# JianCao92/speaker-diarization

Measured on AMD Instinct MI355X. Metric: diarized audio throughput (CD gw/BIC + CL hi/BIC), higher is better.
Workload: dtype f64

## Files before the change

### include/spkd.h

```cpp
#ifndef SPKD_H
#define SPKD_H

#include <stddef.h>
#include <stdint.h>

#ifdef __cplusplus
extern "C" {
#endif

#define SPKD_ABI_VERSION 2
#define SPKD_DIM 39
#define SPKD_REC 820

typedef enum {
    SPKD_OK = 0,
    SPKD_EINVAL = 1,
    SPKD_EHIP = 2,
    SPKD_ENONFINITE = 3,
    SPKD_EOVERFLOW = 4,
    SPKD_ENOMEM = 5
} spkd_status;

typedef enum { SPKD_BIC = 0, SPKD_GLR = 1, SPKD_KL2 = 2, SPKD_KL2_PINV = 3 } spkd_kind;

// ... 165 lines not shown
enum { SPKD_AHC_AUTO = 0, SPKD_AHC_MONO = 1, SPKD_AHC_WIDE = 2 };

typedef struct {
    int32_t variant;
    int32_t kind;
    int32_t max_spk;
    int32_t path;
    double lambdac;
    double threshold;
} spkd_ahc_params;

spkd_status spkd_ahc(spkd_ctx *ctx, const double *d_stats, const int64_t *h_seg_off,
                     int64_t n_problems, const spkd_ahc_params *params,
                     int32_t *h_n_merges, int32_t *h_merge_a, int32_t *h_merge_b,
                     double *h_merge_d, double *h_stat_max, double *h_stat_min);

spkd_status spkd_ahc_matrix(spkd_ctx *ctx, const double *d_stats, int64_t n, const spkd_ahc_params *params,
                            const double *d_matrix, double stat_max_in, double stat_min_in,
                            int32_t *h_n_merges, int32_t *h_merge_a, int32_t *h_merge_b,
                            double *h_merge_d, double *h_stat_max, double *h_stat_min);

spkd_status spkd_ahc_fused(spkd_ctx *ctx, const float *d_frames, int64_t n_frames,
                           const double *d_records, int64_t n_records, int64_t *d_line_index,
                           const int64_t *h_seg_off, int64_t n_problems,
                           const int64_t *h_redo_line, const int64_t *h_redo_begin,
                           const int64_t *h_redo_end, int64_t n_redo,
                           const spkd_ahc_params *params,
                           const int32_t **h_n_merges, const int32_t **h_merge_a,
                           const int32_t **h_merge_b, const double **h_merge_d,
                           const int32_t **h_labels);
// ... 158 lines not shown
```

### speaker-diarization_amd/csrc/spkd_cluster.hpp

```cpp
#pragma once
#include "spkd_device.hpp"
#include "spkd_quad.hpp"
#include "spkd_tri.hpp"
#include "../../include/spkd.h"

namespace spkd {

constexpr double MAXINT_F = 9223372036854775808.0;
constexpr double PEN_UNIT = 39.0 + 0.5 * 39.0 * 40.0;
constexpr int AUX = 3 * DA;
constexpr int ERR_DEGENERATE_MERGE = 2;

__device__ __forceinline__ unsigned long long dkey(double v) {
    unsigned long long b = (unsigned long long)__double_as_longlong(v);
    return (b >> 63) ? ~b : (b | 0x8000000000000000ull);
}
__device__ __forceinline__ double dkey_inv(unsigned long long k) {
    unsigned long long b = (k >> 63) ? (k & 0x7fffffffffffffffull) : ~k;
    return __longlong_as_double((long long)b);
}
template <bool MAXOP>
__device__ __forceinline__ unsigned wave_red_u32(unsigned x) {
    auto op = [](unsigned a, unsigned b) { return MAXOP ? (a > b ? a : b) : (a < b ? a : b); };
    x = op(x, (unsigned)__builtin_amdgcn_update_dpp((int)x, (int)x, 0xB1, 0xf, 0xf, false));
// ... 504 lines not shown
            }
        }
    }
    if (variant == 1 && (kind == SPKD_KL2 ? lane_id() == 0 : L.t == 0)) {
        if (wmax == wmax) atomicMax(stat_max + p, dkey(wmax));
        if (wmin == wmin) atomicMin(stat_min + p, dkey(wmin));
    }
}

constexpr int AHC_WAVES = 8;
constexpr int AHC_TPB = AHC_WAVES * WAVE;

#ifdef SPKD_PROFILE
__device__ unsigned long long g_step_prof[8];
__device__ unsigned long long g_ahc_prof[8];
#endif
constexpr int NO_COL = 0x7fffffff;
constexpr int AHC_MAX_N = 65536;


struct RowMin { double mv; int mc, nc; };

template <class Alive>
__device__ __forceinline__ RowMin scan_row(const double* __restrict__ row, long long N, Alive alive,
                                           long long sub_col, double sub_val, int lane) {
    double mv = __builtin_huge_val();
    int mc = NO_COL, nc = NO_COL;
    for (long long c0 = 0; c0 < N; c0 += 4 * WAVE) {
        double v[4];
        int a[4];
// ... 103 lines not shown
        }
    }
}

template <bool TWO>
__global__ __launch_bounds__(AHC_TPB) void k_ahc(
        double* __restrict__ ex, double* __restrict__ pk, const int64_t* __restrict__ seg_off,
        int variant, int kind, int max_spk, double lambdac, double threshold,
        double* __restrict__ ld, double* __restrict__ aux,
        double* __restrict__ mat, const int64_t* __restrict__ mat_off,
        int32_t* __restrict__ alive, double* __restrict__ tmp,
        double* __restrict__ rmin_all, int32_t* __restrict__ rcache_all,
        int32_t* __restrict__ out_n, int32_t* __restrict__ out_a, int32_t* __restrict__ out_b,
        double* __restrict__ out_d, unsigned long long* stat_max, unsigned long long* stat_min,
        double* __restrict__ final_max, double* __restrict__ final_min, int* err,
        double* pinv_ws) {
    extern __shared__ int32_t ids[];
    __shared__ double ldsA[QREC];
    __shared__ unsigned long long red3[AHC_WAVES][3];
    __shared__ unsigned long long s_masks[AHC_MAX_N / WAVE];
    __shared__ int s_cnt[2];
    __shared__ int s_nids;
    __shared__ int s_next;
    __shared__ double s_tmax[AHC_WAVES];
    const int tid = threadIdx.x, lane = lane_id(), wave = tid >> 6;
    const QuadLane L = quad_lane();
    const int p = blockIdx.x;
    const int64_t off = seg_off[p];
    const long long N = seg_off[p + 1] - off;
    double* Dm = mat + mat_off[p];
    int32_t* al = alive + off;
    double* ldp = ld + off;
    double* tp = tmp + off;
    double* rmin = rmin_all + off;
    int32_t* rarg = rcache_all + 3 * off;
    int32_t* rnan = rarg + N;
    int32_t* dirty = rnan + N;
    for (long long c = tid; c < N; c += AHC_TPB) { al[c] = 1; dirty[c] = 1; }
    __syncthreads();
    long long m = N;
    int n_merges = 0;
    const long long INF_IDX = 0x7fffffffffffffffLL;
// ... 170 lines not shown
                if (kmax != 0ull) atomicMax(stat_max + p, kmax);
                if (kmin != ~0ull) atomicMin(stat_min + p, kmin);
            }
        }
        __syncthreads();
        AHC_TICK(4);
    }
#ifdef SPKD_PROFILE
    if (tid == 0) for (int i = 0; i < 5; ++i) atomicAdd(&g_ahc_prof[2 + i], ahc_acc[i]);
#endif
    const double mx = final_matrix_max(Dm, N, [&](long long c) { return al[c] != 0; }, s_tmax, tid);
    if (tid == 0) {
        out_n[p] = n_merges;
        final_max[p] = mx;
        final_min[p] = fmin;
    }
}

constexpr int STEP_WAVES = 4;
constexpr int STEP_WIDE_FROM = 1024;
constexpr int STEP_PARTNERS = 4 * STEP_WAVES - 1;
constexpr int ALIVE_ROUND = 0x7fffffff;
constexpr int STEP_MAX_N = 16384;
constexpr int STEP_IDX_SHIFT = 14;

struct StepState {
    int32_t done, n_merges;
    long long psa;
    double fmin;
    double diag;
// ... 599 lines not shown
```

### speaker-diarization_amd/csrc/spkd_hip.hip

```cpp
#include <hip/hip_runtime.h>

#include <algorithm>
#include <cmath>
#include <cstddef>
#include <cstdio>
#include <cstdlib>
#include <cstring>
#include <string>
#include <atomic>
#include <thread>
#include <vector>

#include "../../include/spkd.h"
#include "spkd_cd.hpp"
#include "spkd_cluster.hpp"
#include "spkd_device.hpp"
#include "spkd_handoff.hpp"
#include "spkd_merge.hpp"
#include "spkd_stats.hpp"
#include "spkd_post_stats.hpp"
#include "spkd_mfcc.hpp"
#include "spkd_mfcc_batch.hpp"
#include "spkd_resample.hpp"
#include "spkd_vad.hpp"
// ... 14 lines not shown
       PIN_GT_TAB, PIN_GT_OUT, PIN_GT_IDX, PIN_UBM_TAB, PIN_UBM_OUT, PIN_CLR_IN, PIN_CLR_OUT, PIN_MD_SEQS, PIN_MD_TOKENS,
       PIN_FB_TAB, PIN_ID_IN, PIN_ID_OUT, PIN_ACC_TAB, PIN_POST_TAB, N_PIN };
}

struct spkd_ctx {
    int device = 0;
    hipStream_t stream = nullptr;
    bool own_stream = false;
    bool gw_lds_ok = false;
    int rs_lds_cap = 0;
    int gw_waves = 0;
    unsigned long long init_keys[2] = {0ull, ~0ull};
    int step_waves = 0;
    int step_partners = 0;
    int64_t last_gw_items = 0;
    std::string err;
    int* d_err = nullptr;
    unsigned long long* d_counter = nullptr;
    hipEvent_t ev0 = nullptr, ev1 = nullptr;
    float last_ms = 0.f;
    hipEvent_t ka[SPKD_N_TIMERS] = {}, kb[SPKD_N_TIMERS] = {};
    bool kused[SPKD_N_TIMERS] = {};
    float kms[SPKD_N_TIMERS] = {};
    void* slot[N_SLOTS] = {};
    size_t slot_bytes[N_SLOTS] = {};
    void* pinv_ws = nullptr;
    double* pinv_cur = nullptr;
    void* pin[N_PIN] = {};
    size_t pin_bytes[N_PIN] = {};
    std::vector<int64_t> redo_line, redo_begin, redo_end;
// ... 93 lines not shown
template <class Parts>
spkd_status upload_parts(spkd_ctx* c, int slot, std::vector<char>& image, Parts parts) {
    image.resize(parts(Layout()));
    parts(Layout(nullptr, image.data()));
    char* d = nullptr;
    TRY(upload(c, slot, image.data(), image.size(), &d));
    parts(Layout(d));
    return SPKD_OK;
}

struct Call {
    spkd_ctx* const c;
    spkd_status opened;
    int herr = 0;
    bool drained = false;
    explicit Call(spkd_ctx* ctx) : c(ctx) { opened = open(); }
    ~Call() { if (!drained) (void)hipStreamSynchronize(c->stream); }
    spkd_status open() {
        HIPCHK(c, hipSetDevice(c->device));
        for (int i = 0; i < SPKD_N_TIMERS; ++i) c->kused[i] = false;
        HIPCHK(c, hipMemsetAsync(c->d_err, 0, sizeof(int), c->stream));
        HIPCHK(c, hipEventRecord(c->ev0, c->stream));
        return SPKD_OK;
    }

    spkd_status finish() {
        HIPCHK(c, hipEventRecord(c->ev1, c->stream));
        HIPCHK(c, hipMemcpyAsync(&herr, c->d_err, sizeof(int), hipMemcpyDeviceToHost, c->stream));
        HIPCHK(c, hipStreamSynchronize(c->stream));
        drained = true;
        HIPCHK(c, hipEventElapsedTime(&c->last_ms, c->ev0, c->ev1));
        c->kms[0] = c->last_ms;
        for (int i = 1; i < SPKD_N_TIMERS; ++i)
            if (c->kused[i]) HIPCHK(c, hipEventElapsedTime(&c->kms[i], c->ka[i], c->kb[i]));
        if (herr & ERR_SWEEP) return fail(c, SPKD_EHIP, "internal error: growing-window sweep order");
        if (herr & 4) return fail(c, SPKD_EOVERFLOW, "device scratch capacity exceeded");
        if (herr & ERR_DEGENERATE_MERGE) return fail(c, SPKD_EINVAL, "degenerate merge: a diagonal cell was the minimum");
        if (herr & ERR_NONFINITE) return fail(c, SPKD_ENONFINITE, "array must not contain infs or NaNs");
        return SPKD_OK;
    }
};

struct Image { char* base = nullptr; size_t bytes = 0; };
template <class Tab, class Parts>
// ... 106 lines not shown
    c->gw_lds_ok = hipDeviceGetAttribute(&lds_max, hipDeviceAttributeMaxSharedMemoryPerBlock, device) == hipSuccess &&
                   Gw<4>::LDS_BYTES <= lds_max &&
                   hipFuncSetAttribute((const void*)k_gw<8>, hipFuncAttributeMaxDynamicSharedMemorySize, Gw<8>::LDS_BYTES) == hipSuccess &&
                   hipFuncSetAttribute((const void*)k_gw<4>, hipFuncAttributeMaxDynamicSharedMemorySize, Gw<4>::LDS_BYTES) == hipSuccess &&
                   hipFuncSetAttribute((const void*)k_gw<2>, hipFuncAttributeMaxDynamicSharedMemorySize, Gw<2>::LDS_BYTES) == hipSuccess &&
                   hipFuncSetAttribute((const void*)k_gw<1>, hipFuncAttributeMaxDynamicSharedMemorySize, Gw<1>::LDS_BYTES) == hipSuccess;
    c->rs_lds_cap = 64 * 1024;
    if (lds_max > c->rs_lds_cap) {
        const int want = lds_max < RS_LDS_MAX ? lds_max : RS_LDS_MAX;
        if (hipFuncSetAttribute((const void*)k_resample, hipFuncAttributeMaxDynamicSharedMemorySize, want) == hipSuccess)
            c->rs_lds_cap = want;
    }
    if (const char* e = getenv("SPKD_GW_WAVES")) c->gw_waves = atoi(e);
    if (const char* e = getenv("SPKD_STEP_WAVES")) { const int v = atoi(e); c->step_waves = (v == 4 || v == 8) ? v : 0; }
    if (const char* e = getenv("SPKD_STEP_PARTNERS")) { const int v = atoi(e); c->step_partners = (v == 3 || v == 7 || v == 15) ? v : 0; }
    *out = c;
    return SPKD_OK;
}

spkd_status spkd_create(int device, void* stream, spkd_ctx** out) {
    return create_ctx(device, stream, stream != nullptr, out);
}

spkd_status spkd_create_on_stream(int device, void* stream, spkd_ctx** out) {
    return create_ctx(device, stream, true, out);
}

void spkd_destroy(spkd_ctx* c) {
    if (!c) return;
    (void)hipSetDevice(c->device);
    if (c->stream) (void)hipStreamSynchronize(c->stream);
    for (int i = 0; i < N_SLOTS; ++i)
        if (c->slot[i]) (void)hipFree(c->slot[i]);
    if (c->d_err) (void)hipFree(c->d_err);
    if (c->pinv_ws) (void)hipFree(c->pinv_ws);
    for (int i = 0; i < N_PIN; ++i)
        if (c->pin[i]) (void)hipHostFree(c->pin[i]);
    if (c->d_counter) (void)hipFree(c->d_counter);
    if (c->ev0) (void)hipEventDestroy(c->ev0);
    if (c->ev1) (void)hipEventDestroy(c->ev1);
    for (int i = 0; i < SPKD_N_TIMERS; ++i) {
        if (c->ka[i]) (void)hipEventDestroy(c->ka[i]);
        if (c->kb[i]) (void)hipEventDestroy(c->kb[i]);
    }
    if (c->own_stream && c->stream) (void)hipStreamDestroy(c->stream);
    delete c;
// ... 142 lines not shown
namespace {
struct AhcPrep {
    double* ex;
    double* pk;
    double* ld;
    double* aux;
    double* mat;
    int64_t* seg_off;
    int64_t* mat_off;
    unsigned long long* smax;
    unsigned long long* smin;
    int64_t n_total = 0;
    int64_t grid_rows = 0;
    std::vector<char> offs;
    std::vector<char> prob_of;
};

unsigned long long host_dkey(double v) {
    unsigned long long b;
    std::memcpy(&b, &v, sizeof b);
    return (b >> 63) ? ~b : (b | 0x8000000000000000ull);
}

struct MatrixPlan {
    const double* d_init = nullptr;
    double init_max = NAN, init_min = NAN;
    int64_t row_begin = -1, row_end = -1;
    int64_t* d_map = nullptr;
    int64_t n_src = 0;
    const float* d_frames = nullptr;
    int64_t n_frames = 0;
    const int64_t *redo_line = nullptr, *redo_begin = nullptr, *redo_end = nullptr;
    int64_t n_redo = 0;
};

void to_quadrec(spkd_ctx* c, const double* d_stats, int64_t n, double* ex) {
    hipLaunchKernelGGL(k_to_quadrec, dim3((unsigned)n), dim3(256), 0, c->stream, d_stats, n, ex);
}

void cluster_prep(spkd_ctx* c, const double* ex, int64_t n, int kind, double* ld, double* aux) {
    const int64_t per_block = kind == SPKD_KL2 ? PT_WAVES : 4 * PT_WAVES;
    const unsigned blocks = (unsigned)((n + per_block - 1) / per_block);
    hipLaunchKernelGGL(k_cluster_prep, dim3(blocks), dim3(PT_WAVES * WAVE), 0, c->stream, ex, n, kind, ld, aux, c->d_err,
                       c->pinv_cur);
}

spkd_status ahc_prepare(spkd_ctx* c, const double* d_stats, const int64_t* h_seg_off, int64_t n_prob,
                        int variant, int kind, double lambdac, AhcPrep& B, const MatrixPlan& plan = MatrixPlan()) {
    const int64_t n_total = B.n_total = h_seg_off[n_prob];
    const size_t np = (size_t)n_prob;
    std::vector<int64_t> mat_off(np + 1);
    int64_t cells = 0;
    for (int64_t p = 0; p < n_prob; ++p) {
        const int64_t n = h_seg_off[p + 1] - h_seg_off[p];
        if (n < 0) return fail(c, SPKD_EINVAL, "seg_off must be non-decreasing");
        mat_off[(size_t)p] = cells;
        cells += n * n;
    }
    mat_off[np] = cells;
    std::vector<int32_t> prob((size_t)n_total, 0);
    for (int64_t p = 0; p < n_prob; ++p)
        for (int64_t r = h_seg_off[p]; r < h_seg_off[p + 1]; ++r) prob[(size_t)r] = (int32_t)p;
    int32_t *d_prob = nullptr, *d_sched = nullptr;
    {
        const int X = 8;
        std::vector<std::vector<int32_t>> lists(X);
        if (plan.row_begin >= 0) {
            for (int64_t r = plan.row_begin; r < plan.row_end; ++r) lists[(size_t)((r - plan.row_begin) % X)].push_back((int32_t)r);
        } else if (n_prob >= X) {
            std::vector<int64_t> order((size_t)n_prob);
            for (int64_t p = 0; p < n_prob; ++p) order[(size_t)p] = p;
            std::stable_sort(order.begin(), order.end(), [&](int64_t a, int64_t b) {
                return h_seg_off[a + 1] - h_seg_off[a] > h_seg_off[b + 1] - h_seg_off[b];
            });
            double load[X] = {0, 0, 0, 0, 0, 0, 0, 0};
            for (int64_t p : order) {
                int x = 0;
                for (int i = 1; i < X; ++i) if (load[i] < load[x]) x = i;
                const double n = (double)(h_seg_off[p + 1] - h_seg_off[p]);
                load[x] += n * n;
                for (int64_t r = h_seg_off[p]; r < h_seg_off[p + 1]; ++r) lists[x].push_back((int32_t)r);
            }
        } else {
            for (int64_t r = 0; r < n_total; ++r) lists[(size_t)(r % X)].push_back((int32_t)r);
        }
        size_t longest = 0;
        for (auto& l : lists) longest = std::max(longest, l.size());
        B.grid_rows = (int64_t)longest * X;
        std::vector<int32_t> sched((size_t)B.grid_rows, -1);
        for (int x = 0; x < X; ++x)
            for (size_t i = 0; i < lists[x].size(); ++i) sched[i * X + x] = lists[x][i];
        TRY(upload_parts(c, S_AHC_OFF, B.offs, [&](Layout L) {
            return L.part(B.seg_off, np + 1, h_seg_off).part(B.mat_off, np + 1, mat_off.data()).bytes();
        }));
        TRY(upload_parts(c, S_AHC_PROB, B.prob_of, [&](Layout L) {
            return L.part(d_prob, prob.size(), prob.data()).part(d_sched, sched.size(), sched.data()).bytes();
        }));
    }
    const size_t nt = (size_t)n_total;
    TRY(carve(c, scratch, S_AHC_LD, [&](Layout L) { return L.part(B.ld, nt).bytes(); }));
    TRY(carve(c, scratch, S_AHC_AUX, [&](Layout L) { return L.part(B.aux, nt * AUX).bytes(); }));
    TRY(carve(c, scratch, S_AHC_MAT, [&](Layout L) { return L.part(B.mat, (size_t)cells).bytes(); }));
    TRY(carve(c, scratch, S_AHC_MISC, [&](Layout L) { return L.part(B.smax, np).part(B.smin, np).bytes(); }));
    HIPCHK(c, hipMemsetAsync(B.smax, 0x00, (size_t)n_prob * sizeof(unsigned long long), c->stream));
    HIPCHK(c, hipMemsetAsync(B.smin, 0xff, (size_t)n_prob * sizeof(unsigned long long), c->stream));
    if (plan.d_init && n_prob == 1) {
        c->init_keys[0] = plan.init_max == plan.init_max ? host_dkey(plan.init_max) : 0ull;
        c->init_keys[1] = plan.init_min == plan.init_min ? host_dkey(plan.init_min) : ~0ull;
        HIPCHK(c, hipMemcpyAsync(B.smax, &c->init_keys[0], sizeof(unsigned long long), hipMemcpyHostToDevice, c->stream));
        HIPCHK(c, hipMemcpyAsync(B.smin, &c->init_keys[1], sizeof(unsigned long long), hipMemcpyHostToDevice, c->stream));
    }
    TRY(carve(c, scratch, S_AHC_STATS, [&](Layout L) { return L.part(B.ex, nt * QREC).bytes(); }));
    TRY(carve(c, scratch, S_AHC_PACKED, [&](Layout L) { return L.part(B.pk, nt * REC).bytes(); }));
// ... 9 lines not shown
                TRY(set_stats_launch(c, plan.d_frames, plan.n_frames, plan.redo_begin, plan.redo_end, c->redo_sets.data(),
                                     plan.n_redo, plan.n_redo, (double*)d_redo, c->redo_chunks, c->redo_setoff));
                hipLaunchKernelGGL(k_patch_map, dim3((unsigned)((plan.n_redo + 255) / 256)), dim3(256), 0, c->stream,
                                   (const int64_t*)d_rl, plan.n_redo, plan.d_map);
            }
            hipLaunchKernelGGL(k_records_from_map, dim3((unsigned)n_total), dim3(256), 0, c->stream, d_stats, plan.n_src,
                               (const int64_t*)plan.d_map, (const double*)d_redo, plan.n_redo, n_total, B.ex, B.pk, c->d_err);
        } else {
            to_quadrec(c, d_stats, n_total, B.ex);
            HIPCHK(c, hipMemcpyAsync(B.pk, d_stats, (size_t)n_total * REC * sizeof(double), hipMemcpyDeviceToDevice, c->stream));
        }
        {
            Timer t(c, SPKD_T_CLUSTER_PREP);
            cluster_prep(c, B.ex, n_total, kind, B.ld, B.aux);
        }
        auto kmat = kind == SPKD_GLR ? k_matrix<true> : k_matrix<false>;
        if (plan.d_init) {
            HIPCHK(c, hipMemcpyAsync(B.mat, plan.d_init, (size_t)cells * sizeof(double), hipMemcpyDeviceToDevice, c->stream));
        } else if (B.grid_rows > 0) {
            Timer t(c, SPKD_T_MATRIX);
            hipLaunchKernelGGL(kmat, dim3((unsigned)B.grid_rows), dim3(MX_WAVES * WAVE), 0, c->stream,
                               (const double*)B.ex, (const double*)B.pk, (const int64_t*)B.seg_off, (const int32_t*)d_prob,
                               (const int32_t*)d_sched, variant, kind, lambdac,
                               (const double*)B.ld, (const double*)B.aux, B.mat, (const int64_t*)B.mat_off,
                               B.smax, B.smin, c->d_err);
        }
    }
    HIPCHK(c, hipGetLastError());
    return SPKD_OK;
}

double key_to_double(unsigned long long k, bool is_max) {
    if (is_max ? (k == 0ull) : (k == ~0ull)) return std::nan("");
    unsigned long long b = (k >> 63) ? (k & 0x7fffffffffffffffull) : ~k;
    double v;
    std::memcpy(&v, &b, sizeof v);
    return v;
}
}

// ... 192 lines not shown
        return fail(c, SPKD_EINVAL, "null argument");
    if ((P->variant != 1 && P->variant != 2) || bad_kind(P->kind))
        return fail(c, SPKD_EINVAL, "bad variant / kind");
    for (int64_t p = 0; p < n_prob; ++p)
        if (h_seg_off[p + 1] - h_seg_off[p] < 1) return fail(c, SPKD_EINVAL, "empty clustering problem");
    int64_t n_max = 0;
    for (int64_t p = 0; p < n_prob; ++p) n_max = std::max<int64_t>(n_max, h_seg_off[p + 1] - h_seg_off[p]);
    if (n_max > AHC_MAX_N) return fail(c, SPKD_EINVAL, "clustering problem larger than 65536 records");
    int path = P->path;
    if (path != SPKD_AHC_MONO && path != SPKD_AHC_WIDE) path = n_prob <= 64 ? SPKD_AHC_WIDE : SPKD_AHC_MONO;
    const size_t lds = (size_t)(n_max + 4) * sizeof(int32_t);
    if (path == SPKD_AHC_MONO && lds > 150 * 1024) path = SPKD_AHC_WIDE;
    if (path == SPKD_AHC_WIDE && n_max > STEP_MAX_N)
        return fail(c, SPKD_EINVAL, "clustering problem larger than 16384 records (wide merge loop)");
    AhcPrep B;
    std::vector<unsigned long long> kmax((size_t)n_prob), kmin((size_t)n_prob);
    std::vector<double> fmax((size_t)n_prob), fmin((size_t)n_prob);
    Call call(c);
    TRY(call.opened);
    spkd_ahc_params Pk;
    TRY(kernel_params(c, P, Pk));
    TRY(ahc_prepare(c, d_stats, h_seg_off, n_prob, P->variant, P->kind, P->lambdac, B, plan));
    const int64_t n_total = B.n_total;
    const size_t nt = (size_t)n_total, np = (size_t)n_prob;
    double *d_merge_d, *d_tmp, *d_rmin, *d_fmax, *d_fmin;
    int32_t *d_a, *d_b, *d_alive, *d_rcache, *d_n;
    TRY(carve(c, scratch, S_AHC_OUT, [&](Layout L) {
        return L.part(d_merge_d, nt).part(d_tmp, nt).part(d_rmin, nt).part(d_fmax, np).part(d_fmin, np)
            .part(d_a, nt).part(d_b, nt).part(d_alive, nt).part(d_rcache, 3 * nt).part(d_n, np).bytes();
    }));
    if (path == SPKD_AHC_MONO) {
        auto kahc = P->kind == SPKD_GLR ? k_ahc<true> : k_ahc<false>;
        if (lds > 48 * 1024)
            (void)hipFuncSetAttribute((const void*)kahc, hipFuncAttributeMaxDynamicSharedMemorySize, (int)lds);
        Timer t(c, SPKD_T_AHC);
        hipLaunchKernelGGL(kahc, dim3((unsigned)n_prob), dim3(AHC_TPB), lds, c->stream,
                           B.ex, B.pk, (const int64_t*)B.seg_off, P->variant, P->kind, P->max_spk, P->lambdac,
                           P->threshold, B.ld, B.aux, B.mat, (const int64_t*)B.mat_off, d_alive, d_tmp,
                           d_rmin, d_rcache, d_n, d_a, d_b, d_merge_d, B.smax, B.smin, d_fmax, d_fmin, c->d_err,
                           c->pinv_cur);
    } else {
        StepArrays Q;
        void *pe = nullptr, *pp = nullptr;
        TRY(carve(c, scratch, S_STEP_MISC, [&](Layout L) {
            return L.part(Q.sel2, 2 * nt).part(Q.cnt, nt).part(Q.sw, nt).part(Q.state2, 2 * np).part(Q.death, nt).bytes();
        }));
        TRY(scratch(c, S_STEP_EXM, nt * QREC * sizeof(double), &pe));
        TRY(scratch(c, S_STEP_PKM, nt * REC * sizeof(double), &pp));
        Q.ex = B.ex; Q.pk = B.pk; Q.exm = (double*)pe; Q.pkm = (double*)pp;
        Q.n_total = n_total;
        Q.n_prob = (int32_t)n_prob;
        const int step_waves = c->step_waves ? c->step_waves : (n_max > STEP_WIDE_FROM ? 8 : 4);
        const bool glr_k = P->kind == SPKD_GLR;
        using StepKernel = decltype(&k_ahc_step<false, 4, 3>);
        StepKernel kvar[3];
// ... 66 lines not shown
                    h_stat_max, h_stat_min);
}

spkd_status spkd_ahc_matrix(spkd_ctx* c, const double* d_stats, int64_t n, const spkd_ahc_params* P,
                            const double* d_matrix, double stat_max_in, double stat_min_in,
                            int32_t* h_n_merges, int32_t* h_merge_a, int32_t* h_merge_b, double* h_merge_d,
                            double* h_stat_max, double* h_stat_min) {
    if (!c || n < 1) return SPKD_EINVAL;
    if (!d_matrix) return fail(c, SPKD_EINVAL, "ahc_matrix: null matrix");
    const int64_t seg_off[2] = {0, n};
    MatrixPlan plan;
    plan.d_init = d_matrix;
    plan.init_max = stat_max_in;
    plan.init_min = stat_min_in;
    return ahc_impl(c, d_stats, seg_off, 1, P, plan, h_n_merges, h_merge_a, h_merge_b, h_merge_d, h_stat_max, h_stat_min);
}

int64_t spkd_gw_event_capacity(int64_t turn_len, double rate) {
    if (turn_len < 0 || !(rate >= 10.0)) return -1;
    return (int64_t)((double)turn_len / (0.2 * rate)) + 8;
}

int64_t spkd_gw_event_capacity_p(int64_t turn_len, const spkd_cd_params* P) {
    if (turn_len < 0 || !P || !(P->rate >= 10.0) || !(P->winstep >= 1.0)) return -1;
    const double step = std::min(0.2 * P->rate, std::min(0.5 * P->rate, P->winstep));
    return (int64_t)((double)turn_len / step) + 8;
}

int64_t spkd_sw_window_count(int64_t turn_len, double winsize, double winstep) {
    if (!(winstep >= 1.0) || !(winsize >= 1.0)) return -1;
// ... 2157 lines not shown
        for (auto& th : pool) th.join();
    }
    return bad.load() ? SPKD_EINVAL : SPKD_OK;
}

}

#ifdef SPKD_PROFILE
extern "C" int spkd_debug_ahc_prof(unsigned long long* out4) {
    unsigned long long z[8] = {0, 0, 0, 0, 0, 0, 0, 0};
    if (hipMemcpyFromSymbol(out4, HIP_SYMBOL(spkd::g_ahc_prof), sizeof z) != hipSuccess) return 1;
    if (hipMemcpyToSymbol(HIP_SYMBOL(spkd::g_ahc_prof), z, sizeof z) != hipSuccess) return 1;
    return 0;
}

extern "C" int spkd_debug_step_prof(unsigned long long* out8) {
    unsigned long long z[8] = {0, 0, 0, 0, 0, 0, 0, 0};
    if (hipMemcpyFromSymbol(out8, HIP_SYMBOL(spkd::g_step_prof), sizeof z) != hipSuccess) return 1;
    if (hipMemcpyToSymbol(HIP_SYMBOL(spkd::g_step_prof), z, sizeof z) != hipSuccess) return 1;
    return 0;
}

extern "C" int spkd_debug_pass_prof(unsigned long long* out4) {
    unsigned long long z[4] = {0, 0, 0, 0};
    if (hipMemcpyFromSymbol(out4, HIP_SYMBOL(spkd::g_pass_prof), sizeof z) != hipSuccess) return 1;
    if (hipMemcpyToSymbol(HIP_SYMBOL(spkd::g_pass_prof), z, sizeof z) != hipSuccess) return 1;
    return 0;
}

extern "C" int spkd_debug_gw_prof(unsigned long long* out12) {
// ... 7 lines not shown
```

### speaker-diarization_amd/hipabi.py

```python
import ctypes as C
import os

import numpy as np

HERE = os.path.dirname(os.path.abspath(__file__))
LIB_PATH = os.environ.get('SPKD_HIP_LIBRARY') or os.path.join(HERE, 'csrc', 'libspkd_hip.so')

SPKD_OK, SPKD_EINVAL, SPKD_EHIP, SPKD_ENONFINITE, SPKD_EOVERFLOW, SPKD_ENOMEM = range(6)
KINDS = {'BIC': 0, 'GLR': 1, 'KL2': 2, 'KL2P': 3}
WANT_GLR, WANT_KL2, WANT_KL2_PINV = 1, 2, 4
MERGE_NO_AHEAD = 1
TIMERS = {n: i for i, n in enumerate(['call', 'chunk_stats', 'reduce_sets', 'pair_terms',
                                        'cluster_prep', 'matrix', 'ahc', 'gw', 'sw', 'merge',
                                        'vad_shift', 'vad_viterbi', 'vad_backtrack', 'gauss_models', 'gauss_loglik',
                                        'post_stats', 'resample',
                                        'gmm_train', 'gmm_seq_loglik', 'ubm_stats', 'clr_link',
                                        'mindur_viterbi', 'mindur_backtrack', 'fb_posterior',
                                        'ident_scores', 'ident_assign', 'bw_accumulate',
                                        'mfcc_static', 'mfcc_post'])}
VAD_TILE = 32
MINDUR_TILE = 32
FB_TILE = 32
POST_CHUNK = 1024
GAUSS_TILE = 64
# ... 8 lines not shown
MFCC_POST_TILE = 128
MFCC_POST_HALO = 4
MFCC_POST_LDS = 61440
MFCC_CMS_MAX = 272
RESAMPLE_TILE = 2048
RESAMPLE_MAX_CH = 8
RESAMPLE_MAX_HALF = 256
RESAMPLE_MAX_TERM = 1 << 20
RESAMPLE_MAX_TAPS = 1 << 22
RESAMPLE_MAX_SPAN = 33281
REC = 820
DIM = 39

EXPORTS = ['spkd_abi_version', 'spkd_create', 'spkd_create_on_stream', 'spkd_destroy', 'spkd_last_error', 'spkd_sync',
           'spkd_malloc', 'spkd_free', 'spkd_memcpy_h2d', 'spkd_memcpy_d2h', 'spkd_memcpy_d2d',
           'spkd_last_kernel_ms', 'spkd_last_gw_items', 'spkd_set_stats', 'spkd_pair_terms',
           'spkd_distance_matrix', 'spkd_gw_event_capacity', 'spkd_gw_event_capacity_p', 'spkd_gw', 'spkd_gw_ex', 'spkd_gw_fused', 'spkd_gw_batch', 'spkd_ahc_fused', 'spkd_gather_stats', 'spkd_sum_stats', 'spkd_mfcc', 'spkd_mfcc_batch', 'spkd_resample_batch',
           'spkd_sw_window_count', 'spkd_sw', 'spkd_sw_runs', 'spkd_sw_batch', 'spkd_merge_batch', 'spkd_ahc', 'spkd_ahc_matrix', 'spkd_distance_rows', 'spkd_cluster_in', 'spkd_cluster_in_batch', 'spkd_py2_roundtrip',
           'spkd_labels_from_merges', 'spkd_labels_from_merges_batch', 'spkd_count_flags', 'spkd_gw_lines',
           'spkd_gmm_loglik', 'spkd_vad_viterbi', 'spkd_vad_shift_batch', 'spkd_vad_viterbi_batch',
           'spkd_gauss_models', 'spkd_gauss_loglik', 'spkd_gmm_train', 'spkd_gmm_loglik_seq',
           'spkd_ubm_stats', 'spkd_clr_link', 'spkd_mindur_viterbi_batch', 'spkd_fb_posterior_batch',
           'spkd_clr_identify', 'spkd_bw_accumulate', 'spkd_post_stats']


class CdParams(C.Structure):
    _fields_ = [('kind', C.c_int32), ('trace', C.c_int32), ('lambdac', C.c_double),
                ('threshold', C.c_double), ('winsize', C.c_double), ('winstep', C.c_double),
                ('deltaws', C.c_double), ('rate', C.c_double)]


# ... 100 lines not shown
    lib.spkd_abi_version.restype = C.c_int
    lib.spkd_create.argtypes = [C.c_int, vp, P(vp)]
    lib.spkd_create_on_stream.argtypes = [C.c_int, vp, P(vp)]
    lib.spkd_destroy.argtypes = [vp]
    lib.spkd_destroy.restype = None
    lib.spkd_last_error.argtypes = [vp]
    lib.spkd_last_error.restype = C.c_char_p
    lib.spkd_sync.argtypes = [vp]
    lib.spkd_malloc.argtypes = [vp, C.c_size_t, P(vp)]
    lib.spkd_free.argtypes = [vp, vp]
    lib.spkd_memcpy_h2d.argtypes = [vp, vp, vp, C.c_size_t]
    lib.spkd_memcpy_d2h.argtypes = [vp, vp, vp, C.c_size_t]
    lib.spkd_memcpy_d2d.argtypes = [vp, vp, vp, C.c_size_t]
    lib.spkd_last_kernel_ms.argtypes = [vp, C.c_int, P(C.c_float)]
    lib.spkd_last_gw_items.argtypes = [vp, P(C.c_int64)]
    lib.spkd_set_stats.argtypes = [vp, vp, i64, vp, vp, vp, i64, i64, vp]
    lib.spkd_pair_terms.argtypes = [vp, vp, vp, vp, i64, C.c_int, vp]
    lib.spkd_distance_matrix.argtypes = [vp, C.c_int, dbl, vp, i64, vp]
    lib.spkd_gw_event_capacity.argtypes = [i64, dbl]
    lib.spkd_gw_event_capacity.restype = i64
    lib.spkd_gw_event_capacity_p.argtypes = [i64, P(CdParams)]
    lib.spkd_gw_event_capacity_p.restype = i64
    lib.spkd_gw.argtypes = [vp, vp, i64, vp, vp, i64, P(CdParams), vp, vp, vp, vp, vp, vp, vp, vp,
                            vp, i64, P(i64)]
    lib.spkd_gw_ex.argtypes = [vp, vp, i64, vp, vp, i64, P(CdParams), vp, C.c_int, vp, vp, vp, vp, vp, vp,
                               vp, vp, i64, P(i64)]
    lib.spkd_gw_fused.argtypes = [vp, vp, i64, vp, vp, i64, P(CdParams), vp, C.c_int, vp, vp, vp, vp, vp, vp,
                                  vp, vp, vp, i64, P(i64)]
    lib.spkd_gw_batch.argtypes = [vp, vp, i64, vp, vp, i64, P(CdParams), vp, vp, vp, vp, vp, vp, C.c_int, P(GwLinesView)]
    lib.spkd_ahc_fused.argtypes = [vp, vp, i64, vp, i64, vp, vp, i64, vp, vp, vp, i64, P(AhcParams),
# ... 197 lines not shown
    def check(self, st, allow=()):
        if st != SPKD_OK and st not in allow:
            raise SpkdError(st, self.lib.spkd_last_error(self.h).decode())
        return st

    def last_ms(self, which='call'):
        ms = C.c_float()
        self.check(self.lib.spkd_last_kernel_ms(self.h, TIMERS[which], C.byref(ms)))
        return ms.value

    def last_gw_items(self):
        n = C.c_int64()
        self.check(self.lib.spkd_last_gw_items(self.h, C.byref(n)))
        return int(n.value)

    def dev_alloc(self, nbytes):
        p = C.c_void_p()
        self.check(self.lib.spkd_malloc(self.h, nbytes, C.byref(p)))
        return p.value

    def dev_free(self, ptr):
        if ptr:
            self.check(self.lib.spkd_free(self.h, C.c_void_p(ptr)))

    def dev_scratch(self, name, nbytes):
        cache = self.__dict__.setdefault('_dev_scratch', {})
        ptr, cap = cache.get(name, (None, 0))
        if ptr is None or cap < nbytes:
            if ptr is not None:
                self.dev_free(ptr)
# ... 534 lines not shown
```

### speaker-diarization_amd/pipeline.py

```python
import time

import numpy as np

from . import gallery as _gallery
from . import hipabi
from . import resegmentation as _resegmentation
from .recipe import py2_float_str
from .resegmentation import (FB_MAX_SCALED_PENALTY, RESEG, RESEG_CONF, RESEG_GMM, RESEG_MAX_SPEAKERS, RESEG_MD,
                             RESEG_SOFT, RESEG_SOFT_SCALE, resegment_batch)

DIA2_CD = dict(kind='BIC', lambdac=1.0, threshold=0.0, winsize_s=1.0, winstep_s=3.0, deltaws_s=0.1)
DIA2_CL = dict(variant=1, kind='BIC', lambdac=1.3, threshold=0.0, max_spk=0)
SW_CD = dict(method='sw', kind='GLR', lambdac=1.3, threshold=0.0, winsize_s=5.0, winstep_s=0.5, deltaws_s=0.05)
MERGE_CD = dict(method='m', kind='GLR', lambdac=1.3, threshold=0.0, winsize_s=5.0, winstep_s=0.5, deltaws_s=0.05)
LINK_CL = dict(variant=1, kind='BIC', lambdac=1.3, threshold=0.0, max_spk=0)
LINK_CLR = dict(model='clr', components=8, iterations=5, var_floor=0.01, relevance=16.0,
                threshold=-0.5, max_spk=0, ubm_max_frames=2_000_000)


class BatchFile(object):

    def __init__(self, frame_off, n_frames, vad):
        self.frame_off = int(frame_off)
        self.n_frames = int(n_frames)
# ... 151 lines not shown


def _time_stats(ctx, timings, n, begin, end):
    if len(begin):
        timings.setdefault('chunk_stats', []).append(ctx.last_ms('chunk_stats'))
        timings.setdefault('reduce_sets', []).append(ctx.last_ms('reduce_sets'))
    timings['stats_frames'] = int((end - begin).sum())
    timings['stats_sets'] = n
    timings['stats_recomputed'] = len(begin)


def _clustering_done(ctx, timings, seg_off, r):
    if timings is not None:
        for k in ('cluster_prep', 'matrix', 'ahc'):
            timings.setdefault(k, []).append(ctx.last_ms(k))
    if r['status'] == hipabi.SPKD_ENONFINITE:
        raise ValueError('array must not contain infs or NaNs')
    if timings is not None:
        npb = np.diff(seg_off)
        nm = r['n_merges'].astype(np.int64)
        timings['matrix_pairs'] = int((npb * (npb - 1) // 2).sum())
        timings['ahc_pairs'] = int((nm * (npb - 2) - nm * (nm - 1) // 2).sum())


def _cluster_in_done(ctx, timings, seg_off, r):
    if timings is not None:
        for k in ('cluster_prep', 'ahc'):
            timings.setdefault(k, []).append(ctx.last_ms(k))
    if r['status'] == hipabi.SPKD_ENONFINITE:
        raise ValueError('array must not contain infs or NaNs')
# ... 583 lines not shown
```

Baseline: 1482.

## Overlap head-problem merge loops with remaining distance-matrix build on a side stream

Problems are sorted by size and a host cost model picks a head of the largest ones. Their distance-matrix rows are built first, and their AHC merge loops then start on a second stream. That work overlaps with the matrix build and merge loops for the remaining problems on the main stream. The aim is to stop the long serial merge loop of the biggest problem from sitting idle behind the whole matrix kernel. The cost is extra streams, events and schedule tables, a hard-coded per-N² cost model that may pick a head size of zero, and contention for compute units while the two streams run together.

```diff
diff --git a/include/spkd.h b/include/spkd.h
--- a/include/spkd.h
+++ b/include/spkd.h
@@ -203,6 +203,9 @@
                      int64_t n_problems, const spkd_ahc_params *params,
                      int32_t *h_n_merges, int32_t *h_merge_a, int32_t *h_merge_b,
                      double *h_merge_d, double *h_stat_max, double *h_stat_min);
+
+int64_t spkd_ahc_head_rule(const int64_t *h_seg_off, int64_t n_problems);
+spkd_status spkd_last_ahc_head(spkd_ctx *ctx, int64_t *k);
 
 spkd_status spkd_ahc_matrix(spkd_ctx *ctx, const double *d_stats, int64_t n, const spkd_ahc_params *params,
                             const double *d_matrix, double stat_max_in, double stat_min_in,
diff --git a/speaker-diarization_amd/csrc/spkd_cluster.hpp b/speaker-diarization_amd/csrc/spkd_cluster.hpp
--- a/speaker-diarization_amd/csrc/spkd_cluster.hpp
+++ b/speaker-diarization_amd/csrc/spkd_cluster.hpp
@@ -542,6 +542,8 @@
 #ifdef SPKD_PROFILE
 __device__ unsigned long long g_step_prof[8];
 __device__ unsigned long long g_ahc_prof[8];
+constexpr int AHC_SPAN_PROBS = 4096;
+__device__ unsigned long long g_ahc_span[2 * AHC_SPAN_PROBS];
 #endif
 constexpr int NO_COL = 0x7fffffff;
 constexpr int AHC_MAX_N = 65536;
@@ -675,7 +677,7 @@
         int32_t* __restrict__ out_n, int32_t* __restrict__ out_a, int32_t* __restrict__ out_b,
         double* __restrict__ out_d, unsigned long long* stat_max, unsigned long long* stat_min,
         double* __restrict__ final_max, double* __restrict__ final_min, int* err,
-        double* pinv_ws) {
+        double* pinv_ws, const int32_t* __restrict__ prob_of_block) {
     extern __shared__ int32_t ids[];
     __shared__ double ldsA[QREC];
     __shared__ unsigned long long red3[AHC_WAVES][3];
@@ -686,7 +688,10 @@
     __shared__ double s_tmax[AHC_WAVES];
     const int tid = threadIdx.x, lane = lane_id(), wave = tid >> 6;
     const QuadLane L = quad_lane();
-    const int p = blockIdx.x;
+    const int p = prob_of_block ? prob_of_block[blockIdx.x] : (int)blockIdx.x;
+#ifdef SPKD_PROFILE
+    if (tid == 0 && p < AHC_SPAN_PROBS) g_ahc_span[2 * p] = wall_clock64();
+#endif
     const int64_t off = seg_off[p];
     const long long N = seg_off[p + 1] - off;
     double* Dm = mat + mat_off[p];
@@ -887,6 +892,9 @@
         out_n[p] = n_merges;
         final_max[p] = mx;
         final_min[p] = fmin;
+#ifdef SPKD_PROFILE
+        if (p < AHC_SPAN_PROBS) g_ahc_span[2 * p + 1] = wall_clock64();
+#endif
     }
 }
 
diff --git a/speaker-diarization_amd/csrc/spkd_hip.hip b/speaker-diarization_amd/csrc/spkd_hip.hip
--- a/speaker-diarization_amd/csrc/spkd_hip.hip
+++ b/speaker-diarization_amd/csrc/spkd_hip.hip
@@ -6,6 +6,7 @@
 #include <cstdio>
 #include <cstdlib>
 #include <cstring>
+#include <functional>
 #include <string>
 #include <atomic>
 #include <thread>
@@ -52,6 +53,10 @@
     int step_waves = 0;
     int step_partners = 0;
     int64_t last_gw_items = 0;
+    int ahc_head = -1;
+    int64_t last_ahc_head = 0;
+    hipStream_t side = nullptr;
+    hipEvent_t ev_fork = nullptr, ev_join = nullptr;
     std::string err;
     int* d_err = nullptr;
     unsigned long long* d_counter = nullptr;
@@ -175,8 +180,13 @@
     spkd_status opened;
     int herr = 0;
     bool drained = false;
+    bool forked = false, joined = false;
     explicit Call(spkd_ctx* ctx) : c(ctx) { opened = open(); }
-    ~Call() { if (!drained) (void)hipStreamSynchronize(c->stream); }
+    ~Call() {
+        if (drained) return;
+        (void)hipStreamSynchronize(c->stream);
+        if (forked) (void)hipStreamSynchronize(c->side);
+    }
     spkd_status open() {
         HIPCHK(c, hipSetDevice(c->device));
         for (int i = 0; i < SPKD_N_TIMERS; ++i) c->kused[i] = false;
@@ -185,10 +195,29 @@
         return SPKD_OK;
     }
 
+    spkd_status fork() {
+        if (!c->side) HIPCHK(c, hipStreamCreateWithFlags(&c->side, hipStreamNonBlocking));
+        if (!c->ev_fork) HIPCHK(c, hipEventCreateWithFlags(&c->ev_fork, hipEventDisableTiming));
+        if (!c->ev_join) HIPCHK(c, hipEventCreateWithFlags(&c->ev_join, hipEventDisableTiming));
+        HIPCHK(c, hipEventRecord(c->ev_fork, c->stream));
+        forked = true;
+        HIPCHK(c, hipStreamWaitEvent(c->side, c->ev_fork, 0));
+        return SPKD_OK;
+    }
+    spkd_status join() {
+        if (!forked || joined) return SPKD_OK;
+        HIPCHK(c, hipEventRecord(c->ev_join, c->side));
+        HIPCHK(c, hipStreamWaitEvent(c->stream, c->ev_join, 0));
+        joined = true;
+        return SPKD_OK;
+    }
+
     spkd_status finish() {
+        TRY(join());
         HIPCHK(c, hipEventRecord(c->ev1, c->stream));
         HIPCHK(c, hipMemcpyAsync(&herr, c->d_err, sizeof(int), hipMemcpyDeviceToHost, c->stream));
         HIPCHK(c, hipStreamSynchronize(c->stream));
+        if (forked) HIPCHK(c, hipStreamSynchronize(c->side));
         drained = true;
         HIPCHK(c, hipEventElapsedTime(&c->last_ms, c->ev0, c->ev1));
         c->kms[0] = c->last_ms;
@@ -325,6 +354,7 @@
     if (const char* e = getenv("SPKD_GW_WAVES")) c->gw_waves = atoi(e);
     if (const char* e = getenv("SPKD_STEP_WAVES")) { const int v = atoi(e); c->step_waves = (v == 4 || v == 8) ? v : 0; }
     if (const char* e = getenv("SPKD_STEP_PARTNERS")) { const int v = atoi(e); c->step_partners = (v == 3 || v == 7 || v == 15) ? v : 0; }
+    if (const char* e = getenv("SPKD_AHC_HEAD")) { const int v = atoi(e); c->ahc_head = v >= 0 ? v : -1; }
     *out = c;
     return SPKD_OK;
 }
@@ -341,6 +371,12 @@
     if (!c) return;
     (void)hipSetDevice(c->device);
     if (c->stream) (void)hipStreamSynchronize(c->stream);
+    if (c->side) {
+        (void)hipStreamSynchronize(c->side);
+        (void)hipStreamDestroy(c->side);
+    }
+    if (c->ev_fork) (void)hipEventDestroy(c->ev_fork);
+    if (c->ev_join) (void)hipEventDestroy(c->ev_join);
     for (int i = 0; i < N_SLOTS; ++i)
         if (c->slot[i]) (void)hipFree(c->slot[i]);
     if (c->d_err) (void)hipFree(c->d_err);
@@ -513,7 +549,49 @@
     int64_t grid_rows = 0;
     std::vector<char> offs;
     std::vector<char> prob_of;
+    int64_t head_k = 0;
+    int64_t grid_head = 0;
+    int64_t n_max_head = 0, n_max_rest = 0;
+    int32_t *d_prob = nullptr, *d_sched = nullptr, *d_sched_head = nullptr, *d_block_head = nullptr, *d_block_rest = nullptr;
+    int variant = 1, kind = 0;
+    double lambdac = 0.0;
 };
+
+constexpr int N_XCD = 8;
+void deal_to_xcds(const int64_t* h_seg_off, const std::vector<int64_t>& order, std::vector<int32_t>& sched,
+                  std::vector<int32_t>* by_xcd = nullptr) {
+    const int X = N_XCD;
+    std::vector<std::vector<int32_t>> lists(X), probs(X);
+    if ((int64_t)order.size() >= X) {
+        double load[X] = {0, 0, 0, 0, 0, 0, 0, 0};
+        for (int64_t p : order) {
+            int x = 0;
+            for (int i = 1; i < X; ++i) if (load[i] < load[x]) x = i;
+            const double n = (double)(h_seg_off[p + 1] - h_seg_off[p]);
+            load[x] += n * n;
+            probs[x].push_back((int32_t)p);
+            for (int64_t r = h_seg_off[p]; r < h_seg_off[p + 1]; ++r) lists[x].push_back((int32_t)r);
+        }
+    } else {
+        std::vector<int64_t> asc(order);
+        std::sort(asc.begin(), asc.end());
+        int64_t i = 0;
+        for (size_t k = 0; k < order.size(); ++k) {
+            probs[k].push_back((int32_t)order[k]);
+            for (int64_t r = h_seg_off[asc[k]]; r < h_seg_off[asc[k] + 1]; ++r) lists[(size_t)(i++ % X)].push_back((int32_t)r);
+        }
+    }
+    size_t longest = 0;
+    for (auto& l : lists) longest = std::max(longest, l.size());
+    sched.assign(longest * X, -1);
+    for (int x = 0; x < X; ++x)
+        for (size_t i = 0; i < lists[x].size(); ++i) sched[i * X + x] = lists[x][i];
+    if (by_xcd) {
+        by_xcd->clear();
+        for (size_t i = 0; by_xcd->size() < order.size(); ++i)
+            for (int x = 0; x < X; ++x) if (i < probs[x].size()) by_xcd->push_back(probs[x][i]);
+    }
+}
 
 unsigned long long host_dkey(double v) {
     unsigned long long b;
@@ -544,6 +622,40 @@
                        c->pinv_cur);
 }
 
+void matrix_launch(spkd_ctx* c, const AhcPrep& B, const int32_t* d_sched, int64_t grid) {
+    if (grid <= 0) return;
+    auto kmat = B.kind == SPKD_GLR ? k_matrix<true> : k_matrix<false>;
+    hipLaunchKernelGGL(kmat, dim3((unsigned)grid), dim3(MX_WAVES * WAVE), 0, c->stream,
+                       (const double*)B.ex, (const double*)B.pk, (const int64_t*)B.seg_off, (const int32_t*)B.d_prob,
+                       d_sched, B.variant, B.kind, B.lambdac,
+                       (const double*)B.ld, (const double*)B.aux, B.mat, (const int64_t*)B.mat_off,
+                       B.smax, B.smin, c->d_err);
+}
+
+constexpr int AHC_HEAD_ROUND = 32;
+constexpr double AHC_MS_PER_N2 = 2.095e-4;
+constexpr double MATRIX_MS_PER_N2 = 6.00e-7;
+constexpr int AHC_HEAD_MAX = 32;
+constexpr int AHC_RULE_CUS = 256;
+int64_t ahc_head_rule(const std::vector<int64_t>& n, int cus) {
+    const int64_t n_prob = (int64_t)n.size();
+    if (n_prob < 16) return 0;
+    auto t = [](int64_t N) { return AHC_MS_PER_N2 * (double)N * (double)N; };
+    double sum_all = 0.0;
+    for (int64_t N : n) sum_all += (double)N * (double)N;
+    const double stage0 = MATRIX_MS_PER_N2 * sum_all + t(n[0]);
+    double best = stage0, sum_head = 0.0;
+    int64_t best_k = 0;
+    for (int64_t k = 1; k <= std::min<int64_t>(AHC_HEAD_MAX, n_prob) && k < cus; ++k) {
+        sum_head += (double)n[(size_t)k - 1] * (double)n[(size_t)k - 1];
+        const double m_head = MATRIX_MS_PER_N2 * sum_head, m_rest = MATRIX_MS_PER_N2 * (sum_all - sum_head);
+        const double rest = k < n_prob ? m_rest * cus / (double)(cus - k) + t(n[(size_t)k]) : 0.0;
+        const double stage = m_head + std::max(t(n[0]), rest);
+        if (k % AHC_HEAD_ROUND == 0 && stage < best) { best = stage; best_k = k; }
+    }
+    return stage0 - best < 0.01 * stage0 ? 0 : best_k;
+}
+
 spkd_status ahc_prepare(spkd_ctx* c, const double* d_stats, const int64_t* h_seg_off, int64_t n_prob,
                         int variant, int kind, double lambdac, AhcPrep& B, const MatrixPlan& plan = MatrixPlan()) {
     const int64_t n_total = B.n_total = h_seg_off[n_prob];
@@ -560,42 +672,41 @@
     std::vector<int32_t> prob((size_t)n_total, 0);
     for (int64_t p = 0; p < n_prob; ++p)
         for (int64_t r = h_seg_off[p]; r < h_seg_off[p + 1]; ++r) prob[(size_t)r] = (int32_t)p;
-    int32_t *d_prob = nullptr, *d_sched = nullptr;
     {
-        const int X = 8;
-        std::vector<std::vector<int32_t>> lists(X);
+        std::vector<int32_t> sched, sched_head, block_head, block_rest;
         if (plan.row_begin >= 0) {
-            for (int64_t r = plan.row_begin; r < plan.row_end; ++r) lists[(size_t)((r - plan.row_begin) % X)].push_back((int32_t)r);
-        } else if (n_prob >= X) {
+            const int64_t rows = plan.row_end - plan.row_begin;
+            sched.assign((size_t)((rows + N_XCD - 1) / N_XCD * N_XCD), -1);
+            for (int64_t i = 0; i < rows; ++i) sched[(size_t)i] = (int32_t)(plan.row_begin + i);
+        } else {
             std::vector<int64_t> order((size_t)n_prob);
             for (int64_t p = 0; p < n_prob; ++p) order[(size_t)p] = p;
             std::stable_sort(order.begin(), order.end(), [&](int64_t a, int64_t b) {
                 return h_seg_off[a + 1] - h_seg_off[a] > h_seg_off[b + 1] - h_seg_off[b];
             });
-            double load[X] = {0, 0, 0, 0, 0, 0, 0, 0};
-            for (int64_t p : order) {
-                int x = 0;
-                for (int i = 1; i < X; ++i) if (load[i] < load[x]) x = i;
-                const double n = (double)(h_seg_off[p + 1] - h_seg_off[p]);
-                load[x] += n * n;
-                for (int64_t r = h_seg_off[p]; r < h_seg_off[p + 1]; ++r) lists[x].push_back((int32_t)r);
+            const std::vector<int64_t> head(order.begin(), order.begin() + B.head_k), rest(order.begin() + B.head_k, order.end());
+            deal_to_xcds(h_seg_off, rest, sched);
+            if (B.head_k > 0) {
+                deal_to_xcds(h_seg_off, head, sched_head, &block_head);
+                std::vector<char> in_head((size_t)n_prob, 0);
+                for (int64_t p : head) in_head[(size_t)p] = 1;
+                for (int64_t p = 0; p < n_prob; ++p) if (!in_head[(size_t)p]) block_rest.push_back((int32_t)p);
+                B.n_max_head = h_seg_off[head[0] + 1] - h_seg_off[head[0]];
+                B.n_max_rest = rest.empty() ? 0 : h_seg_off[rest[0] + 1] - h_seg_off[rest[0]];
             }
-        } else {
-            for (int64_t r = 0; r < n_total; ++r) lists[(size_t)(r % X)].push_back((int32_t)r);
-        }
-        size_t longest = 0;
-        for (auto& l : lists) longest = std::max(longest, l.size());
-        B.grid_rows = (int64_t)longest * X;
-        std::vector<int32_t> sched((size_t)B.grid_rows, -1);
-        for (int x = 0; x < X; ++x)
-            for (size_t i = 0; i < lists[x].size(); ++i) sched[i * X + x] = lists[x][i];
+        }
+        B.grid_rows = (int64_t)sched.size();
+        B.grid_head = (int64_t)sched_head.size();
         TRY(upload_parts(c, S_AHC_OFF, B.offs, [&](Layout L) {
             return L.part(B.seg_off, np + 1, h_seg_off).part(B.mat_off, np + 1, mat_off.data()).bytes();
         }));
         TRY(upload_parts(c, S_AHC_PROB, B.prob_of, [&](Layout L) {
-            return L.part(d_prob, prob.size(), prob.data()).part(d_sched, sched.size(), sched.data()).bytes();
+            return L.part(B.d_prob, prob.size(), prob.data()).part(B.d_sched, sched.size(), sched.data())
+                .part(B.d_sched_head, sched_head.size(), sched_head.data()).part(B.d_block_head, block_head.size(), block_head.data())
+                .part(B.d_block_rest, block_rest.size(), block_rest.data()).bytes();
         }));
     }
+    B.variant = variant; B.kind = kind; B.lambdac = lambdac;
     const size_t nt = (size_t)n_total;
     TRY(carve(c, scratch, S_AHC_LD, [&](Layout L) { return L.part(B.ld, nt).bytes(); }));
     TRY(carve(c, scratch, S_AHC_AUX, [&](Layout L) { return L.part(B.aux, nt * AUX).bytes(); }));
@@ -635,16 +746,14 @@
             Timer t(c, SPKD_T_CLUSTER_PREP);
             cluster_prep(c, B.ex, n_total, kind, B.ld, B.aux);
         }
-        auto kmat = kind == SPKD_GLR ? k_matrix<true> : k_matrix<false>;
         if (plan.d_init) {
             HIPCHK(c, hipMemcpyAsync(B.mat, plan.d_init, (size_t)cells * sizeof(double), hipMemcpyDeviceToDevice, c->stream));
+        } else if (B.head_k > 0) {
+            (void)hipEventRecord(c->ka[SPKD_T_MATRIX], c->stream);
+            matrix_launch(c, B, B.d_sched_head, B.grid_head);
         } else if (B.grid_rows > 0) {
             Timer t(c, SPKD_T_MATRIX);
-            hipLaunchKernelGGL(kmat, dim3((unsigned)B.grid_rows), dim3(MX_WAVES * WAVE), 0, c->stream,
-                               (const double*)B.ex, (const double*)B.pk, (const int64_t*)B.seg_off, (const int32_t*)d_prob,
-                               (const int32_t*)d_sched, variant, kind, lambdac,
-                               (const double*)B.ld, (const double*)B.aux, B.mat, (const int64_t*)B.mat_off,
-                               B.smax, B.smin, c->d_err);
+            matrix_launch(c, B, B.d_sched, B.grid_rows);
         }
     }
     HIPCHK(c, hipGetLastError());
@@ -867,6 +976,11 @@
     if (path == SPKD_AHC_WIDE && n_max > STEP_MAX_N)
         return fail(c, SPKD_EINVAL, "clustering problem larger than 16384 records (wide merge loop)");
     AhcPrep B;
+    c->last_ahc_head = 0;
+    if (path == SPKD_AHC_MONO && !plan.d_init && plan.row_begin < 0 && P->kind != SPKD_KL2_PINV) {
+        B.head_k = c->ahc_head >= 0 ? std::min<int64_t>(c->ahc_head, n_prob) : spkd_ahc_head_rule(h_seg_off, n_prob);
+        c->last_ahc_head = B.head_k;
+    }
     std::vector<unsigned long long> kmax((size_t)n_prob), kmin((size_t)n_prob);
     std::vector<double> fmax((size_t)n_prob), fmin((size_t)n_prob);
     Call call(c);
@@ -886,12 +1000,29 @@
         auto kahc = P->kind == SPKD_GLR ? k_ahc<true> : k_ahc<false>;
         if (lds > 48 * 1024)
             (void)hipFuncSetAttribute((const void*)kahc, hipFuncAttributeMaxDynamicSharedMemorySize, (int)lds);
-        Timer t(c, SPKD_T_AHC);
-        hipLaunchKernelGGL(kahc, dim3((unsigned)n_prob), dim3(AHC_TPB), lds, c->stream,
-                           B.ex, B.pk, (const int64_t*)B.seg_off, P->variant, P->kind, P->max_spk, P->lambdac,
-                           P->threshold, B.ld, B.aux, B.mat, (const int64_t*)B.mat_off, d_alive, d_tmp,
-                           d_rmin, d_rcache, d_n, d_a, d_b, d_merge_d, B.smax, B.smin, d_fmax, d_fmin, c->d_err,
-                           c->pinv_cur);
+        auto merge_loops = [&](hipStream_t on, int64_t grid, const int32_t* blocks, int64_t largest) {
+            hipLaunchKernelGGL(kahc, dim3((unsigned)grid), dim3(AHC_TPB), (size_t)(largest + 4) * sizeof(int32_t), on,
+                               B.ex, B.pk, (const int64_t*)B.seg_off, P->variant, P->kind, P->max_spk, P->lambdac,
+                               P->threshold, B.ld, B.aux, B.mat, (const int64_t*)B.mat_off, d_alive, d_tmp,
+                               d_rmin, d_rcache, d_n, d_a, d_b, d_merge_d, B.smax, B.smin, d_fmax, d_fmin, c->d_err,
+                               c->pinv_cur, blocks);
+        };
+        if (B.head_k > 0) {
+            TRY(call.fork());
+            (void)hipEventRecord(c->ka[SPKD_T_AHC], c->side);
+            merge_loops(c->side, B.head_k, B.d_block_head, B.n_max_head);
+            matrix_launch(c, B, B.d_sched, B.grid_rows);
+            (void)hipEventRecord(c->kb[SPKD_T_MATRIX], c->stream);
+            c->kused[SPKD_T_MATRIX] = true;
+            if (n_prob > B.head_k) merge_loops(c->stream, n_prob - B.head_k, B.d_block_rest, B.n_max_rest);
+            HIPCHK(c, hipGetLastError());
+            TRY(call.join());
+            (void)hipEventRecord(c->kb[SPKD_T_AHC], c->stream);
+            c->kused[SPKD_T_AHC] = true;
+        } else {
+            Timer t(c, SPKD_T_AHC);
+            merge_loops(c->stream, n_prob, nullptr, n_max);
+        }
     } else {
         StepArrays Q;
         void *pe = nullptr, *pp = nullptr;
@@ -988,6 +1119,20 @@
     plan.init_max = stat_max_in;
     plan.init_min = stat_min_in;
     return ahc_impl(c, d_stats, seg_off, 1, P, plan, h_n_merges, h_merge_a, h_merge_b, h_merge_d, h_stat_max, h_stat_min);
+}
+
+spkd_status spkd_last_ahc_head(spkd_ctx* c, int64_t* k) {
+    if (!c || !k) return SPKD_EINVAL;
+    *k = c->last_ahc_head;
+    return SPKD_OK;
+}
+
+int64_t spkd_ahc_head_rule(const int64_t* h_seg_off, int64_t n_prob) {
+    if (!h_seg_off || n_prob < 0) return -1;
+    std::vector<int64_t> sizes((size_t)n_prob);
+    for (int64_t p = 0; p < n_prob; ++p) sizes[(size_t)p] = h_seg_off[p + 1] - h_seg_off[p];
+    std::sort(sizes.begin(), sizes.end(), std::greater<int64_t>());
+    return ahc_head_rule(sizes, AHC_RULE_CUS);
 }
 
 int64_t spkd_gw_event_capacity(int64_t turn_len, double rate) {
@@ -3175,6 +3320,16 @@
     return 0;
 }
 
+extern "C" int spkd_debug_ahc_span(unsigned long long* out, int n_prob, int* khz) {
+    if (n_prob < 0 || n_prob > spkd::AHC_SPAN_PROBS) return 1;
+    std::vector<unsigned long long> z(2 * (size_t)spkd::AHC_SPAN_PROBS, 0ull);
+    if (hipMemcpyFromSymbol(out, HIP_SYMBOL(spkd::g_ahc_span), 2 * (size_t)n_prob * sizeof(unsigned long long)) != hipSuccess) return 1;
+    if (hipMemcpyToSymbol(HIP_SYMBOL(spkd::g_ahc_span), z.data(), z.size() * sizeof(unsigned long long)) != hipSuccess) return 1;
+    int dev = 0;
+    if (hipGetDevice(&dev) != hipSuccess || hipDeviceGetAttribute(khz, hipDeviceAttributeWallClockRate, dev) != hipSuccess) return 1;
+    return 0;
+}
+
 extern "C" int spkd_debug_step_prof(unsigned long long* out8) {
     unsigned long long z[8] = {0, 0, 0, 0, 0, 0, 0, 0};
     if (hipMemcpyFromSymbol(out8, HIP_SYMBOL(spkd::g_step_prof), sizeof z) != hipSuccess) return 1;
diff --git a/speaker-diarization_amd/hipabi.py b/speaker-diarization_amd/hipabi.py
--- a/speaker-diarization_amd/hipabi.py
+++ b/speaker-diarization_amd/hipabi.py
@@ -46,7 +46,7 @@
 
 EXPORTS = ['spkd_abi_version', 'spkd_create', 'spkd_create_on_stream', 'spkd_destroy', 'spkd_last_error', 'spkd_sync',
            'spkd_malloc', 'spkd_free', 'spkd_memcpy_h2d', 'spkd_memcpy_d2h', 'spkd_memcpy_d2d',
-           'spkd_last_kernel_ms', 'spkd_last_gw_items', 'spkd_set_stats', 'spkd_pair_terms',
+           'spkd_last_kernel_ms', 'spkd_last_gw_items', 'spkd_last_ahc_head', 'spkd_ahc_head_rule', 'spkd_set_stats', 'spkd_pair_terms',
            'spkd_distance_matrix', 'spkd_gw_event_capacity', 'spkd_gw_event_capacity_p', 'spkd_gw', 'spkd_gw_ex', 'spkd_gw_fused', 'spkd_gw_batch', 'spkd_ahc_fused', 'spkd_gather_stats', 'spkd_sum_stats', 'spkd_mfcc', 'spkd_mfcc_batch', 'spkd_resample_batch',
            'spkd_sw_window_count', 'spkd_sw', 'spkd_sw_runs', 'spkd_sw_batch', 'spkd_merge_batch', 'spkd_ahc', 'spkd_ahc_matrix', 'spkd_distance_rows', 'spkd_cluster_in', 'spkd_cluster_in_batch', 'spkd_py2_roundtrip',
            'spkd_labels_from_merges', 'spkd_labels_from_merges_batch', 'spkd_count_flags', 'spkd_gw_lines',
@@ -177,6 +177,9 @@
     lib.spkd_memcpy_d2d.argtypes = [vp, vp, vp, C.c_size_t]
     lib.spkd_last_kernel_ms.argtypes = [vp, C.c_int, P(C.c_float)]
     lib.spkd_last_gw_items.argtypes = [vp, P(C.c_int64)]
+    lib.spkd_last_ahc_head.argtypes = [vp, P(C.c_int64)]
+    lib.spkd_ahc_head_rule.argtypes = [vp, i64]
+    lib.spkd_ahc_head_rule.restype = i64
     lib.spkd_set_stats.argtypes = [vp, vp, i64, vp, vp, vp, i64, i64, vp]
     lib.spkd_pair_terms.argtypes = [vp, vp, vp, vp, i64, C.c_int, vp]
     lib.spkd_distance_matrix.argtypes = [vp, C.c_int, dbl, vp, i64, vp]
@@ -404,6 +407,11 @@
         self.check(self.lib.spkd_last_gw_items(self.h, C.byref(n)))
         return int(n.value)
 
+    def last_ahc_head(self):
+        k = C.c_int64()
+        self.check(self.lib.spkd_last_ahc_head(self.h, C.byref(k)))
+        return int(k.value)
+
     def dev_alloc(self, nbytes):
         p = C.c_void_p()
         self.check(self.lib.spkd_malloc(self.h, nbytes, C.byref(p)))
diff --git a/speaker-diarization_amd/pipeline.py b/speaker-diarization_amd/pipeline.py
--- a/speaker-diarization_amd/pipeline.py
+++ b/speaker-diarization_amd/pipeline.py
@@ -189,6 +189,7 @@
     if timings is not None:
         for k in ('cluster_prep', 'matrix', 'ahc'):
             timings.setdefault(k, []).append(ctx.last_ms(k))
+        timings['ahc_head'] = ctx.last_ahc_head()
     if r['status'] == hipabi.SPKD_ENONFINITE:
         raise ValueError('array must not contain infs or NaNs')
     if timings is not None:
```

After: 1543 (median of 6 runs). 1.04x the previous value.
